# amy-leaf/Recommender-System-using-Apache-Spark-MLlib-

Hardware: AMD Instinct MI355X
Metric: ratings/sec per ALS iteration (rank 64) (higher is better)
Workload: dtype f32-grade (split-f16 x3 MFMA, fp32 accumulate)

## Files before the change

recommender-system-using-apache-spark-mllib-_amd/csrc/gram_solve.hip:

```cpp
#include "als_common.h"
#include "task_order.h"

#include <algorithm>
#include <utility>

namespace als {

typedef float floatx4 __attribute__((ext_vector_type(4)));

constexpr int kYtyTasks = 512;
__host__ __device__ inline int64_t yty_chunk(int64_t n) {
  const int64_t c = (n + kYtyTasks - 1) / kYtyTasks;
  return c < 32 ? 32 : (c + 31) / 32 * 32;
}
constexpr int kRescueGrid = 64;
constexpr float kCondMax = 32.f;
constexpr float kCondMaxImplicit = 8.f;
constexpr int kMaxRank = 128;

template <int CN>
struct Cfg {
  static constexpr int KP = 16 * CN;
  static constexpr int NT = CN * (CN + 1) / 2;
  static constexpr int NP = KP * (KP + 1) / 2;
// ... 302 lines not shown
    const float c1 = alpha * fabsf(rv);
    w = v ? sc * __builtin_sqrtf(c1) : 0.f;
    b = (v && rv > 0.f) ? 1.f + c1 : 0.f;
  } else {
    w = v ? sc : 0.f;
    b = v ? rv : 0.f;
  }
  st_c[lane] = ci;
  st_w[lane] = w;
  st_b[lane] = b;
}

template <int CN, class TS>
__device__ __forceinline__ void split_issue(SplitStep<TS::NC>& s, const int* __restrict__ st_c,
                                            int h, const float* __restrict__ Y, int ld, int d0,
                                            int k) {
  const int q = (threadIdx.x & 63) >> 4;
  const int o = 32 * h + 8 * q;
  const int4 c0 = *reinterpret_cast<const int4*>(st_c + o);
  const int4 c1 = *reinterpret_cast<const int4*>(st_c + o + 4);
  const int ids[8] = {c0.x, c0.y, c0.z, c0.w, c1.x, c1.y, c1.z, c1.w};
#pragma unroll
  for (int j = 0; j < 8; ++j)
    TS::load_clamped(Y + (int64_t)(ids[j] >= 0 ? ids[j] : 0) * ld, s.y[j], d0, ld);
}

template <class TS, bool IMPLICIT>
__device__ __forceinline__ void split_prepare(const SplitStep<TS::NC>& s,
                                              const float* __restrict__ st_w,
                                              const float* __restrict__ st_b, int h,
                                              uint32_t (&hi)[TS::NC][4], uint32_t (&lo)[TS::NC][4],
                                              float (&bf)[TS::NRA]) {
  const int o = 32 * h + 8 * ((threadIdx.x & 63) >> 4);
  const float4 w0 = *reinterpret_cast<const float4*>(st_w + o);
  const float4 w1 = *reinterpret_cast<const float4*>(st_w + o + 4);
  const float4 b0 = *reinterpret_cast<const float4*>(st_b + o);
  const float4 b1 = *reinterpret_cast<const float4*>(st_b + o + 4);
  const float w[8] = {w0.x, w0.y, w0.z, w0.w, w1.x, w1.y, w1.z, w1.w};
  const float b[8] = {b0.x, b0.y, b0.z, b0.w, b1.x, b1.y, b1.z, b1.w};
#pragma unroll
  for (int c = 0; c < TS::NR; ++c)
#pragma unroll
    for (int j = 0; j < 8; ++j) bf[c] = fmaf(b[j], s.y[j][c], bf[c]);
#pragma unroll
  for (int c = 0; c < TS::NC; ++c)
#pragma unroll
    for (int p = 0; p < 4; ++p)
      split_pair_w(s.y[2 * p][c], w[2 * p], s.y[2 * p + 1][c], w[2 * p + 1], hi[c][p], lo[c][p]);
}

template <class TS>
__device__ __forceinline__ void split_mfma(const uint32_t (&hi)[TS::NC][4],
                                           const uint32_t (&lo)[TS::NC][4],
                                           floatx4 (&acc)[TS::N]) {
  static_for<TS::N>([&](auto ti) {
    constexpr int tt = decltype(ti)::value;
    constexpr int a = TS::l1(tt), b = TS::l2(tt);
    const half8v ha = as_h8(hi[a]), hb = as_h8(hi[b]);
    acc[tt] = __builtin_amdgcn_mfma_f32_16x16x32_f16(ha, hb, acc[tt], 0, 0, 0);
    acc[tt] = __builtin_amdgcn_mfma_f32_16x16x32_f16(ha, as_h8(lo[b]), acc[tt], 0, 0, 0);
    acc[tt] = __builtin_amdgcn_mfma_f32_16x16x32_f16(as_h8(lo[a]), hb, acc[tt], 0, 0, 0);
  });
}

template <int CN, bool IMPLICIT, class TS = FullTiles<CN>>
__device__ __forceinline__ void gram_accumulate_split(
    const int32_t* __restrict__ col, const float* __restrict__ val, int64_t pb, int64_t pe,
    const float* __restrict__ Y, int ld, int k, float alpha, float sc,
    floatx4 (&acc)[TS::N], float (&bf)[TS::NRA], int& npos, int* __restrict__ st) {
  const int lane = threadIdx.x & 63, m = lane & 15;
  const int d0 = m * CN;
  int* st_c = st;
  float* st_w = reinterpret_cast<float*>(st + 64);
  float* st_b = reinterpret_cast<float*>(st + 128);
  if (pe <= pb) return;
  auto load_idx = [&](int64_t base, int& ci, float& rv) {
    ci = -1;
    rv = 0.f;
    if (base + lane < pe) {
      ci = col[base + lane];
      rv = val[base + lane];
    }
  };
  const int64_t n = pe - pb;
  const int nsteps = (int)((n + 31) >> 5);
  int ci_n, ci_c;
  float rv_n, rv_c;
  load_idx(pb, ci_c, rv_c);
  load_idx(pb + 64, ci_n, rv_n);
  stage_weights<IMPLICIT>(st_c, st_w, st_b, ci_c, rv_c, sc, alpha);
  if constexpr (IMPLICIT) npos += __popcll(__ballot(ci_c >= 0 && rv_c > 0.f));
  wave_lds_sync();
  SplitStep<TS::NC> sA;
  split_issue<CN, TS>(sA, st_c, 0, Y, ld, d0, k);
  float bp[TS::NRA];
#pragma unroll
  for (int c = 0; c < TS::NRA; ++c) bp[c] = 0.f;
  for (int s = 0; s < nsteps; ++s) {
    uint32_t hi[TS::NC][4], lo[TS::NC][4];
    split_prepare<TS, IMPLICIT>(sA, st_w, st_b, s & 1, hi, lo, bp);
    const int s1 = s + 1;
    if (s1 < nsteps) {
      if ((s1 & 1) == 0) {
        stage_weights<IMPLICIT>(st_c, st_w, st_b, ci_n, rv_n, sc, alpha);
        if constexpr (IMPLICIT) npos += __popcll(__ballot(ci_n >= 0 && rv_n > 0.f));
        wave_lds_sync();
        load_idx(pb + 64 * (int64_t)((s1 >> 1) + 1), ci_n, rv_n);
      }
      split_issue<CN, TS>(sA, st_c, s1 & 1, Y, ld, d0, k);
    }
    split_mfma<TS>(hi, lo, acc);
    if (s & 1) {
#pragma unroll
      for (int c = 0; c < TS::NRA; ++c) {
        bf[c] += bp[c];
        bp[c] = 0.f;
      }
    }
  }
#pragma unroll
  for (int c = 0; c < TS::NRA; ++c) bf[c] += bp[c];
}

__device__ __forceinline__ uint32_t split_word(float t) {
  const _Float16 h = (_Float16)t;
  const _Float16 l = (_Float16)(t - (float)h);
  return (uint32_t)__builtin_bit_cast(unsigned short, h) |
         ((uint32_t)__builtin_bit_cast(unsigned short, l) << 16);
}

template <int NC>
struct PreStep {
  uint32_t w[8][NC];
  uint32_t r[8];
};

template <class TS>
__device__ __forceinline__ void pre_issue(PreStep<TS::NC>& s, const int* __restrict__ st_c,
                                          const uint32_t* __restrict__ st_r, int h,
                                          const uint32_t* __restrict__ base, uint32_t kp) {
  const int q = (threadIdx.x & 63) >> 4;
  const int o = 32 * h + 8 * q;
  const int4 c0 = *reinterpret_cast<const int4*>(st_c + o);
  const int4 c1 = *reinterpret_cast<const int4*>(st_c + o + 4);
  const uint4 r0 = *reinterpret_cast<const uint4*>(st_r + o);
  const uint4 r1 = *reinterpret_cast<const uint4*>(st_r + o + 4);
  const int ids[8] = {c0.x, c0.y, c0.z, c0.w, c1.x, c1.y, c1.z, c1.w};
  s.r[0] = r0.x; s.r[1] = r0.y; s.r[2] = r0.z; s.r[3] = r0.w;
  s.r[4] = r1.x; s.r[5] = r1.y; s.r[6] = r1.z; s.r[7] = r1.w;
#pragma unroll
  for (int j = 0; j < 8; ++j) TS::load_pre(base + (uint64_t)(uint32_t)ids[j] * kp, s.w[j]);
}

template <class TS>
__device__ __forceinline__ void pre_operands(const PreStep<TS::NC>& s, uint32_t rsel,
                                             uint32_t (&hi)[TS::NC][4], uint32_t (&lo)[TS::NC][4],
                                             uint32_t (&rb)[4]) {
#pragma unroll
  for (int c = 0; c < TS::NC; ++c)
#pragma unroll
    for (int p = 0; p < 4; ++p) {
      hi[c][p] = __builtin_amdgcn_perm(s.w[2 * p + 1][c], s.w[2 * p][c], 0x05040100u);
      lo[c][p] = __builtin_amdgcn_perm(s.w[2 * p + 1][c], s.w[2 * p][c], 0x07060302u);
    }
#pragma unroll
  for (int p = 0; p < 4; ++p) rb[p] = __builtin_amdgcn_perm(s.r[2 * p + 1], s.r[2 * p], rsel);
}

template <class TS>
__device__ __forceinline__ void pin_operands(uint32_t (&hi)[TS::NC][4], uint32_t (&lo)[TS::NC][4],
                                             uint32_t (&rb)[4]) {
#pragma unroll
  for (int c = 0; c < TS::NC; ++c)
#pragma unroll
    for (int p = 0; p < 4; ++p) asm volatile("" : "+v"(hi[c][p]), "+v"(lo[c][p]));
  if constexpr (TS::NR > 0) {
#pragma unroll
    for (int p = 0; p < 4; ++p) asm volatile("" : "+v"(rb[p]));
  }
  asm volatile("" ::: "memory");
}

template <class TS>
__device__ __forceinline__ void pre_mfma(const uint32_t (&hi)[TS::NC][4],
                                         const uint32_t (&lo)[TS::NC][4], const uint32_t (&rb)[4],
                                         floatx4 (&acc)[TS::N], floatx4 (&accb)[TS::NRA]) {
  split_mfma<TS>(hi, lo, acc);
  const half8v b = as_h8(rb);
#pragma unroll
  for (int c = 0; c < TS::NR; ++c) {
    accb[c] = __builtin_amdgcn_mfma_f32_16x16x32_f16(as_h8(hi[c]), b, accb[c], 0, 0, 0);
    accb[c] = __builtin_amdgcn_mfma_f32_16x16x32_f16(as_h8(lo[c]), b, accb[c], 0, 0, 0);
  }
}

template <class TS>
__device__ __forceinline__ void gram_accumulate_pre(
    const int32_t* __restrict__ col, const float* __restrict__ val, int64_t pb, int64_t pe,
    const uint32_t* __restrict__ Ysp, uint32_t kp, int zero_row, float sr, int d0,
    floatx4 (&acc)[TS::N], floatx4 (&accb)[TS::NRA], int* __restrict__ st, float& rmax) {
  const int lane = threadIdx.x & 63, m = lane & 15;
  int* st_c = st;
  uint32_t* st_r = reinterpret_cast<uint32_t*>(st + 64);
  if (pe <= pb) return;
  const uint32_t rsel = m == 0 ? 0x05040100u : (m == 1 ? 0x07060302u : 0x0C0C0C0Cu);
  const uint32_t* base = Ysp + d0;
  auto load_idx = [&](int64_t b, int& ci, float& rv) {
    ci = zero_row;
    rv = 0.f;
    if (b + lane < pe) {
      ci = col[b + lane];
      rv = val[b + lane];
    }
  };
  auto stage = [&](int ci, float rv) {
    st_c[lane] = ci;
    st_r[lane] = split_word(sr * rv);
    rmax = fmaxf(rmax, __builtin_fabsf(rv));
    wave_lds_sync();
  };
  const int nsteps = (int)((pe - pb + 31) >> 5);
  int ci, ci_n;
  float rv, rv_n;
  load_idx(pb, ci, rv);
  load_idx(pb + 64, ci_n, rv_n);
  stage(ci, rv);
  PreStep<TS::NC> s;
  pre_issue<TS>(s, st_c, st_r, 0, base, kp);
  for (int t = 0; t < nsteps; ++t) {
    uint32_t hi[TS::NC][4], lo[TS::NC][4], rb[4];
    pre_operands<TS>(s, rsel, hi, lo, rb);
    pin_operands<TS>(hi, lo, rb);
    if (t & 1) {
      stage(ci_n, rv_n);
      load_idx(pb + 64 * (int64_t)((t >> 1) + 2), ci_n, rv_n);
    }
    pre_issue<TS>(s, st_c, st_r, (t + 1) & 1, base, kp);
    pre_mfma<TS>(hi, lo, rb, acc, accb);
  }
}

template <class TS>
__device__ __forceinline__ void gram_accumulate_pre2(
    const int32_t* __restrict__ col, const float* __restrict__ val, int64_t pb, int64_t pe,
    const uint32_t* __restrict__ Ysp, uint32_t kp, int zero_row, float sr, int d0,
    floatx4 (&acc)[TS::N], floatx4 (&accb)[TS::NRA], int* __restrict__ st, float& rmax) {
  const int lane = threadIdx.x & 63, m = lane & 15;
  if (pe <= pb) return;
  const uint32_t rsel = m == 0 ? 0x05040100u : (m == 1 ? 0x07060302u : 0x0C0C0C0Cu);
  const uint32_t* base = Ysp + d0;
  auto load_idx = [&](int64_t b, int& ci, float& rv) {
    ci = zero_row;
    rv = 0.f;
    if (b + lane < pe) {
      ci = col[b + lane];
      rv = val[b + lane];
    }
  };
  auto stage = [&](int slot, int ci, float rv) {
    st[128 * slot + lane] = ci;
    reinterpret_cast<uint32_t*>(st + 128 * slot + 64)[lane] = split_word(sr * rv);
    rmax = fmaxf(rmax, __builtin_fabsf(rv));
    wave_lds_sync();
  };
  auto issue = [&](PreStep<TS::NC>& s, int step) {
    const int slot = (step >> 1) & 1;
    pre_issue<TS>(s, st + 128 * slot, reinterpret_cast<const uint32_t*>(st + 128 * slot + 64),
                  step & 1, base, kp);
  };
  const int nsteps = (int)((pe - pb + 31) >> 5);
  int ci0, ci1, ci_n;
  float rv0, rv1, rv_n;
  load_idx(pb, ci0, rv0);
  load_idx(pb + 64, ci1, rv1);
  load_idx(pb + 128, ci_n, rv_n);
  stage(0, ci0, rv0);
  stage(1, ci1, rv1);
  PreStep<TS::NC> s0, s1;
  issue(s0, 0);
  issue(s1, 1);
  auto body = [&](PreStep<TS::NC>& s, int t) {
    uint32_t hi[TS::NC][4], lo[TS::NC][4], rb[4];
    pre_operands<TS>(s, rsel, hi, lo, rb);
    pin_operands<TS>(hi, lo, rb);
    if (t & 1) {
      stage((t >> 1) & 1, ci_n, rv_n);
      load_idx(pb + 64 * (int64_t)((t >> 1) + 3), ci_n, rv_n);
    }
    issue(s, t + 2);
    pre_mfma<TS>(hi, lo, rb, acc, accb);
  };
  for (int t = 0; t < nsteps; t += 2) {
    body(s0, t);
    if (t + 1 < nsteps) body(s1, t + 1);
  }
}

template <class TS>
__device__ __forceinline__ void rhs_from_tiles(const floatx4 (&accb)[TS::NRA], float scale,
                                               float (&bt)[TS::NRA]) {
  const int lane = threadIdx.x & 63, q = lane >> 4, m = lane & 15;
  const int src = (m >> 2) << 4;
  const int rr = m & 3;
#pragma unroll
  for (int c = 0; c < TS::NRA; ++c) {
    float v[4];
#pragma unroll
    for (int r = 0; r < 4; ++r) v[r] = __shfl(accb[c][r] + __shfl_xor(accb[c][r], 1), src);
    const float x = rr == 0 ? v[0] : (rr == 1 ? v[1] : (rr == 2 ? v[2] : v[3]));
    bt[c] = (c < TS::NR && q == 0) ? x * scale : 0.f;
  }
}

__global__ __launch_bounds__(256) void split_table_kernel(const float* __restrict__ Y,
                                                          int64_t n_src, int ld, int k,
                                                          int kp4_shift,
                                                          const float* __restrict__ scal,
                                                          uint4* __restrict__ Ysp) {
  const float sy = ldexpf(1.f, split_exponent(scal[0]));
  const int64_t total = (n_src + 1) << kp4_shift;
  for (int64_t i = (int64_t)blockIdx.x * 256 + threadIdx.x; i < total;
       i += (int64_t)gridDim.x * 256) {
    const int64_t row = i >> kp4_shift;
    const int d = 4 * (int)(i & ((1 << kp4_shift) - 1));
    float4 v = make_float4(0.f, 0.f, 0.f, 0.f);
    if (row < n_src && d + 4 <= ld) v = *reinterpret_cast<const float4*>(Y + row * ld + d);
    uint4 w;
    w.x = d + 0 < k ? split_word(sy * v.x) : 0u;
    w.y = d + 1 < k ? split_word(sy * v.y) : 0u;
    w.z = d + 2 < k ? split_word(sy * v.z) : 0u;
    w.w = d + 3 < k ? split_word(sy * v.w) : 0u;
    Ysp[i] = w;
  }
}

__device__ __forceinline__ void decode_task(int t, int n_chunks, int n_light, int& chunk,
                                            int& light) {
  const int P = n_chunks < n_light ? n_chunks : n_light;
  chunk = -1;
  light = -1;
  if (t < 2 * P) {
    if (t & 1) light = t >> 1;
    else chunk = t >> 1;
  } else if (n_chunks > P) {
    chunk = t - P;
  } else {
    light = t - P;
  }
}

template <int CN>
__device__ __forceinline__ void tile_ij(int c1, int c2, int r, int& i, int& j) {
  const int lane = threadIdx.x & 63, q = lane >> 4, m = lane & 15;
  i = (4 * q + r) * CN + c1;
  j = m * CN + c2;
}

template <int CN, class T>
__device__ __forceinline__ void pack_gram(const double (&a64)[Cfg<CN>::NT][4], T* __restrict__ P) {
  int tt = 0;
#pragma unroll
  for (int c1 = 0; c1 < CN; ++c1) {
#pragma unroll
    for (int c2 = c1; c2 < CN; ++c2) {
#pragma unroll
      for (int r = 0; r < 4; ++r) {
        int i, j;
        tile_ij<CN>(c1, c2, r, i, j);
        const int hi = i > j ? i : j, lo = i > j ? j : i;
        P[hi * (hi + 1) / 2 + lo] = (T)a64[tt][r];
      }
      ++tt;
    }
  }
}

__device__ __forceinline__ float rcp_t(float d) { return __builtin_amdgcn_rcpf(d); }
__device__ __forceinline__ double rcp_t(double d) {
  double y = __builtin_amdgcn_rcp(d);
  y = fma(fma(-d, y, 1.0), y, y);
  return fma(fma(-d, y, 1.0), y, y);
}
__device__ __forceinline__ float readlane_t(float v, int l) {
  return __builtin_bit_cast(float, __builtin_amdgcn_readlane(__builtin_bit_cast(int, v), l));
}
__device__ __forceinline__ double readlane_t(double v, int l) { return readlane_f64(v, l); }

template <int CN>
struct PanelLds {
  static constexpr int NB = CN, NT = CN * (CN + 1) / 2, CS = 18;
  static constexpr int T = 0, Z = NT * 16 * CS, D = Z + 16 * NB, X = D + 16 * NB,
                       SIZE = X + 16 * NB;
};

__host__ __device__ constexpr int tile_index(int nb, int i, int j) {
  return i * nb - i * (i - 1) / 2 + (j - i);
}

template <int CN>
__device__ __forceinline__ void regularise_f32(floatx4 (&A)[Cfg<CN>::NT], float lam, int k) {
  int tt = 0;
#pragma unroll
  for (int c1 = 0; c1 < CN; ++c1) {
#pragma unroll
    for (int c2 = c1; c2 < CN; ++c2) {
      if (c1 == c2) {
#pragma unroll
        for (int r = 0; r < 4; ++r) {
          int i, j;
          tile_ij<CN>(c1, c2, r, i, j);
          if (i == j) A[tt][r] = (i < k) ? A[tt][r] + lam : 1.f;
        }
      }
      ++tt;
    }
  }
}

template <int P>
__device__ __forceinline__ float gate_above(float x) {
  float r;
  uint64_t m;
  asm volatile("s_lshl_b64 %1, -1, %2\n\ts_nop 0\n\tv_cndmask_b32_e64 %0, 0, %3, %1"
               : "=v"(r), "=&s"(m)
               : "i"(P + 1), "v"(x));
  return r;
}

template <int P>
__device__ __forceinline__ float put_lane(float v, float s) {
  asm volatile("s_nop 1\n\tv_writelane_b32 %0, %1, %2" : "+v"(v) : "s"(s), "i"(P));
  return v;
}

template <int N>
__device__ __forceinline__ void pivot_broadcast(const float (&R)[N], float rb, int p,
                                                float (&a)[N], float& bp) {
  const int addr = p << 2;
#pragma unroll
  for (int i = p; i < N; ++i)
    a[i] = __builtin_bit_cast(float,
                              __builtin_amdgcn_ds_bpermute(addr, __builtin_bit_cast(int, R[i])));
  bp = __builtin_bit_cast(float, __builtin_amdgcn_ds_bpermute(addr, __builtin_bit_cast(int, rb)));
}

template <int N>
__device__ __forceinline__ void pivot_update(float (&R)[N], const float (&a)[N], int p, float f) {
  const float2v nf = {-f, -f};
#pragma unroll
  for (int i = (p + 1) & ~1; i < N; i += 2) {
    const float2v r = __builtin_elementwise_fma((float2v){a[i], a[i + 1]}, nf,
                                                (float2v){R[i], R[i + 1]});
    R[i] = r[0];
    R[i + 1] = r[1];
// ... 653 lines not shown
  });
  bool fin = true;
#pragma unroll
  for (int c = 0; c < NB; ++c) fin = fin && (xcol[c] - xcol[c] == 0.f);
  rmin = fminf(rmin, dpp_f<0xB1>(rmin));
  rmax = fmaxf(rmax, dpp_f<0xB1>(rmax));
  rmin = fminf(rmin, dpp_f<0x4E>(rmin));
  rmax = fmaxf(rmax, dpp_f<0x4E>(rmax));
  rmin = fminf(rmin, dpp_f<0x141>(rmin));
  rmax = fmaxf(rmax, dpp_f<0x141>(rmax));
  rmin = fminf(rmin, dpp_f<0x140>(rmin));
  rmax = fmaxf(rmax, dpp_f<0x140>(rmax));
  return dmin > 0.f && rmin > 0.f && rmax <= cond_max * rmin && __ballot(!fin) == 0;
}

template <int NB, bool SPLIT = kW1SplitSchur<NB>>
__device__ __forceinline__ bool w1_solve(floatx4 (&A)[NB * (NB + 1) / 2], float (&bcol)[NB],
                                         float* __restrict__ lds, int k,
                                         float* __restrict__ xrow, int ld,
                                         float cond_max = kCondMax) {
  float xcol[NB];
  const bool ok = w1_solve_x<NB, SPLIT>(A, bcol, lds, k, xcol, cond_max);
  const int lane = threadIdx.x & 63, m = lane & 15;
  if (lane < 16) {
#pragma unroll
    for (int c = 0; c < NB; ++c) {
      const int d = m * NB + c;
      if (d < ld) xrow[d] = (d < k && ok) ? xcol[c] : 0.f;
    }
  }
  return ok;
}

constexpr int kIrSteps = 3;
constexpr float kIrConv = 3e-4f;
constexpr float kIrDiverge = 0.1f;

struct IrArgs {
  const int32_t* col;
  const float* val;
  const float* Y;
  int64_t pb, pe;
  float alpha;
};

template <int CN>
struct IrLds {
  static constexpr int XS = PanelLds<CN>::SIZE, GS = XS + 128, CC = GS + 128, RV = CC + 64,
                       DX = RV + 16 * CN, SIZE = DX + 16 * CN;
  static_assert(XS % 4 == 0, "fp64 alignment");
};

__device__ __forceinline__ double implicit_residual(const IrArgs& a, int ld, int k,
                                                    const double* __restrict__ yty, double lam_n,
                                                    const double* __restrict__ xs,
                                                    double* __restrict__ gs, int* __restrict__ cc) {
  const int lane = threadIdx.x & 63;
  double r = 0.0;
  for (int64_t base = a.pb; base < a.pe; base += 64) {
    const int nb = (int)(a.pe - base < 64 ? a.pe - base : 64);
    double g = 0.0;
    int c = 0;
    if (lane < nb) {
      c = a.col[base + lane];
      const double rv = (double)a.val[base + lane];
      const float* y = a.Y + (int64_t)c * ld;
      double s0 = 0.0, s1 = 0.0;
      for (int d = 0; d < k; d += 4) {
        const float4 v = *reinterpret_cast<const float4*>(y + d);
        s0 = fma((double)v.x, xs[d], s0);
        s1 = fma((double)v.y, xs[d + 1], s1);
        s0 = fma((double)v.z, xs[d + 2], s0);
        s1 = fma((double)v.w, xs[d + 3], s1);
      }
      const double c1 = (double)a.alpha * fabs(rv);
      g = (rv > 0.0 ? 1.0 + c1 : 0.0) - c1 * (s0 + s1);
    }
    gs[lane] = g;
    cc[lane] = c;
    wave_lds_sync();
    if (lane < k) {
#pragma unroll 8
      for (int j = 0; j < nb; ++j) r = fma(gs[j], (double)a.Y[(int64_t)cc[j] * ld + lane], r);
    }
    wave_lds_sync();
  }
  if (lane < k) {
    for (int e = 0; e < k; ++e) {
      const int hi = lane > e ? lane : e, lo = lane > e ? e : lane;
      r = fma(-yty[hi * (hi + 1) / 2 + lo], xs[e], r);
    }
    r = fma(-lam_n, xs[lane], r);
  }
  return r;
}

template <int CN>
__device__ __forceinline__ bool panel_refine(float* __restrict__ lds, const IrArgs& a, int ld,
                                             int k, const double* __restrict__ yty,
                                             double lam_n) {
  typedef PanelLds<CN> Lo;
  typedef IrLds<CN> Ir;
  float* Xv = lds + Lo::X;
  float* Zv = lds + Lo::Z;
  const float* Dv = lds + Lo::D;
  double* xs = reinterpret_cast<double*>(lds + Ir::XS);
  double* gs = reinterpret_cast<double*>(lds + Ir::GS);
  int* cc = reinterpret_cast<int*>(lds + Ir::CC);
  float* Rv = lds + Ir::RV;
  float* DX = lds + Ir::DX;
  const int lane = threadIdx.x & 63;
  const int pl = (lane % CN) * 16 + lane / CN;
  bool conv = false;
  for (int it = 0; it < kIrSteps; ++it) {
    xs[lane] = lane < k ? (double)Xv[pl] : 0.0;
    wave_lds_sync();
    const double r = implicit_residual(a, ld, k, yty, lam_n, xs, gs, cc);
    if (lane < 16 * CN) Rv[pl] = lane < k ? (float)r : 0.f;
    wave_lds_sync();
    block_fwd_subst<Lo::CS>(CN, lds + Lo::T, Rv, Zv);
    block_back_subst<Lo::CS>(CN, lds + Lo::T, Zv, Dv, DX);
    float nd = 0.f, nx = 0.f;
    if (lane < 16 * CN) {
      const float dx = DX[lane];
      const float xn = Xv[lane] + dx;
      Xv[lane] = xn;
      nd = dx * dx;
      nx = xn * xn;
    }
    wave_lds_sync();
    for (int o = 32; o > 0; o >>= 1) {
      nd += __shfl_xor(nd, o);
      nx += __shfl_xor(nx, o);
    }
    if (nd <= (kIrConv * kIrConv) * nx) {
      conv = true;
      break;
    }
    if (!(nd <= (kIrDiverge * kIrDiverge) * nx)) break;
  }
  return conv;
}

template <int CN, bool IMPLICIT = false>
struct SmemBytes {
  static constexpr int value =
      (int)sizeof(float) * (IMPLICIT ? IrLds<CN>::SIZE : PanelLds<CN>::SIZE);
};
template <bool IMPLICIT>
struct SmemBytes<8, IMPLICIT> {
  static constexpr int value = (int)sizeof(float) * W1Lds::SIZE;
};

__device__ __forceinline__ float shfl_xor_t(float v, int m) { return __shfl_xor(v, m); }
__device__ __forceinline__ double shfl_xor_t(double v, int m) { return shfl_xor_f64(v, m); }

template <int CN, bool IMPLICIT, class AccT>
__device__ __forceinline__ void finish_and_solve(AccT (&tot)[Cfg<CN>::NT][4], AccT (&bt)[CN],
                                                 int64_t n_reg, unsigned char* smem, int k,
                                                 float reg, const double* __restrict__ yty,
                                                 float* __restrict__ xrow, int ld, int row,
                                                 RescueList rl, const IrArgs& ir) {
  constexpr int NT = Cfg<CN>::NT;
  float bq[CN];
  const int m = threadIdx.x & 15;
#pragma unroll
  for (int c = 0; c < CN; ++c) {
    AccT v = bt[c];
    v += shfl_xor_t(v, 16);
    v += shfl_xor_t(v, 32);
    bq[c] = m * CN + c < k ? (float)v : 0.f;
  }
  floatx4 A[NT];
  int tt = 0;
#pragma unroll
  for (int c1 = 0; c1 < CN; ++c1) {
#pragma unroll
    for (int c2 = c1; c2 < CN; ++c2) {
#pragma unroll
      for (int r = 0; r < 4; ++r) {
        if constexpr (IMPLICIT) {
          int i, j;
          tile_ij<CN>(c1, c2, r, i, j);
          const int hi = i > j ? i : j, lo = i > j ? j : i;
          A[tt][r] = (float)((double)tot[tt][r] + yty[hi * (hi + 1) / 2 + lo]);
        } else {
          A[tt][r] = (float)tot[tt][r];
        }
        int i, j;
        tile_ij<CN>(c1, c2, r, i, j);
        if (i >= k || j >= k) A[tt][r] = 0.f;
      }
      ++tt;
    }
  }
  regularise_f32<CN>(A, (float)((double)reg * (double)n_reg), k);
  float* lds = reinterpret_cast<float*>(smem);
  if constexpr (IMPLICIT) {
    bool ok = panel_ldl_solve<CN, false, false>(A, bq, lds, k, xrow, ld);
    if (ok) ok = panel_refine<CN>(lds, ir, ld, k, yty, (double)reg * (double)n_reg);
    panel_store_x<CN>(lds + PanelLds<CN>::X, k, ok, xrow, ld);
    if (!ok) rescue_append(rl, row);
  } else {
    const bool ok = panel_ldl_solve<CN>(A, bq, lds, k, xrow, ld);
    if (!ok) rescue_append(rl, row);
  }
}

template <int N, int NRA>
struct Slot {
  static constexpr int SIZE = (N * 4 + NRA + 1) * 64;
};

template <int N, int NRA, class AccT>
__device__ __forceinline__ void store_slot(double* __restrict__ slot, const AccT (&tot)[N][4],
                                           const AccT (&bt)[NRA], float npos) {
  const int lane = threadIdx.x & 63;
#pragma unroll
  for (int t = 0; t < N; ++t)
#pragma unroll
    for (int r = 0; r < 4; ++r) slot[(t * 4 + r) * 64 + lane] = (double)tot[t][r];
#pragma unroll
  for (int c = 0; c < NRA; ++c) slot[(N * 4 + c) * 64 + lane] = (double)bt[c];
  slot[(N * 4 + NRA) * 64 + lane] = (double)npos;
}

template <int N, int NRA>
__device__ __forceinline__ void add_slot(const double* __restrict__ slot, double (&a64)[N][4],
                                         double (&b64)[NRA], int& npos) {
  const int lane = threadIdx.x & 63;
#pragma unroll
  for (int t = 0; t < N; ++t)
#pragma unroll
    for (int r = 0; r < 4; ++r) a64[t][r] += slot[(t * 4 + r) * 64 + lane];
#pragma unroll
  for (int c = 0; c < NRA; ++c) b64[c] += slot[(N * 4 + c) * 64 + lane];
  npos += (int)slot[(N * 4 + NRA) * 64 + lane];
}

template <int N, int NRA>
__device__ __forceinline__ void store_slot_f32(float* __restrict__ slot, const float (&tot)[N][4],
                                               const float (&bt)[NRA], float npos) {
  const int lane = threadIdx.x & 63;
#pragma unroll
  for (int t = 0; t < N; ++t)
#pragma unroll
    for (int r = 0; r < 4; ++r) slot[(t * 4 + r) * 64 + lane] = tot[t][r];
#pragma unroll
  for (int c = 0; c < NRA; ++c) slot[(N * 4 + c) * 64 + lane] = bt[c];
  slot[(N * 4 + NRA) * 64 + lane] = npos;
}

template <int N, int NRA>
__device__ __forceinline__ void add_slot_f32(const float* __restrict__ slot, double (&a64)[N][4],
                                             double (&b64)[NRA], int& npos) {
  const int lane = threadIdx.x & 63;
#pragma unroll
  for (int t = 0; t < N; ++t)
#pragma unroll
    for (int r = 0; r < 4; ++r) a64[t][r] += (double)slot[(t * 4 + r) * 64 + lane];
#pragma unroll
  for (int c = 0; c < NRA; ++c) b64[c] += (double)slot[(N * 4 + c) * 64 + lane];
  npos += (int)slot[(N * 4 + NRA) * 64 + lane];
}

template <int N, int NRA, class AccT>
__device__ __forceinline__ void zero_acc(AccT (&tot)[N][4], AccT (&bt)[NRA]) {
#pragma unroll
  for (int t = 0; t < N; ++t)
#pragma unroll
    for (int r = 0; r < 4; ++r) tot[t][r] = AccT(0);
#pragma unroll
  for (int c = 0; c < NRA; ++c) bt[c] = AccT(0);
}

template <bool ADD_YTY, int NB = kW1NB, bool SPLIT = kW1SplitSchur<NB>>
__device__ __forceinline__ void w1_finish_and_solve(floatx4 (&A)[NB * (NB + 1) / 2],
                                                    float scale, float (&bt)[NB], int64_t n_reg,
                                                    const float* __restrict__ ytyC,
                                                    unsigned char* smem, int k, float reg,
                                                    float* __restrict__ xrow, int ld, int row,
                                                    RescueList rl, float cond_max = kCondMax);

template <int CN, bool IMPLICIT>
__global__ __launch_bounds__(64, IMPLICIT ? 2 : 3) void gram_solve_kernel(
    const int64_t* __restrict__ row_ptr, const int32_t* __restrict__ col,
    const float* __restrict__ val, const int32_t* __restrict__ light_rows,
    const int32_t* __restrict__ chunk_row, const int64_t* __restrict__ chunk_begin,
    const int64_t* __restrict__ chunk_end, int32_t n_chunks, int32_t n_light,
    const float* __restrict__ Y, float* __restrict__ X, int ld, int k, float reg, float alpha,
    const double* __restrict__ yty, float* __restrict__ slots, int32_t* __restrict__ status,
    const float* __restrict__ scal, const uint32_t* __restrict__ Ysp, int32_t kp,
    int32_t zero_row, RescueList rl) {
  constexpr int NT = Cfg<CN>::NT;
  __shared__ __attribute__((aligned(16))) unsigned char smem[SmemBytes<CN, IMPLICIT>::value];
  floatx4 acc[NT];
#pragma unroll
  for (int t = 0; t < NT; ++t) acc[t] = floatx4{0.f, 0.f, 0.f, 0.f};
  float tot[NT][4], bt[CN];
#pragma unroll
  for (int c = 0; c < CN; ++c) bt[c] = 0.f;
  int npos = 0;
  int chunk, light;
  if constexpr (!IMPLICIT && CN == 4) decode_task_merged(blockIdx.x, n_chunks, n_light, chunk, light);
  else decode_task(blockIdx.x, n_chunks, n_light, chunk, light);
  int64_t pb, pe;
  int row = -1;
  if (chunk >= 0) {
    pb = chunk_begin[chunk];
    pe = chunk_end[chunk];
  } else {
    row = light_rows[light];
    pb = row_ptr[row];
    pe = row_ptr[row + 1];
  }
  float inv2;
  float rmax = 0.f;
  if constexpr (IMPLICIT) {
    const int e = split_exponent(scal[0] * __builtin_sqrtf(alpha * scal[1]));
    inv2 = ldexpf(1.f, -2 * e);
    gram_accumulate_split<CN, true>(col, val, pb, pe, Y, ld, k, alpha, ldexpf(1.f, e), acc, bt,
                                    npos, reinterpret_cast<int*>(smem));
  } else {
    const int ey = split_exponent(scal[0]), er = split_exponent(scal[1]);
    inv2 = ldexpf(1.f, -2 * ey);
    floatx4 accb[CN];
#pragma unroll
    for (int c = 0; c < CN; ++c) accb[c] = floatx4{0.f, 0.f, 0.f, 0.f};
    gram_accumulate_pre<FullTiles<CN>>(col, val, pb, pe, Ysp, (uint32_t)kp, zero_row,
                                       ldexpf(1.f, er), (threadIdx.x & 15) * CN, acc, accb,
                                       reinterpret_cast<int*>(smem), rmax);
    rhs_from_tiles<FullTiles<CN>>(accb, ldexpf(1.f, -ey - er), bt);
    rmax *= ldexpf(1.f, er);
    if (chunk < 0 && (window_miss(diag_max_lane<CN>(acc), (float)(pe - pb), rmax) ||
                      rank_deficient_illcond<CN>(acc, inv2, pe - pb, k, reg))) {
      rescue_append(rl, row);
      return;
    }
  }
#pragma unroll
  for (int t = 0; t < NT; ++t)
#pragma unroll
    for (int r = 0; r < 4; ++r) tot[t][r] = acc[t][r] * inv2;
  if (chunk >= 0) {
    store_slot_f32<NT, CN>(slots + (int64_t)chunk * Cfg<CN>::SLOT, tot, bt,
                           IMPLICIT ? (float)npos : rmax);
    return;
  }
  __syncthreads();
  const int64_t n_reg = IMPLICIT ? (int64_t)npos : (pe - pb);
  if constexpr (!IMPLICIT && CN == 4) {
    static_assert(W1LdsT<4>::SIZE <= PanelLds<4>::SIZE, "W1<4> LDS");
    w1_finish_and_solve<false, 4, false>(acc, inv2, bt, n_reg, nullptr, smem, k, reg,
                                  X + (int64_t)row * ld, ld, row, rl);
  } else {
    finish_and_solve<CN, IMPLICIT, float>(tot, bt, n_reg, smem, k, reg, yty,
                                          X + (int64_t)row * ld, ld, row, rl,
                                          IrArgs{col, val, Y, pb, pe, alpha});
  }
}

__device__ __forceinline__ void block_absmax_publish(float m, unsigned* __restrict__ out) {
  for (int o = 32; o > 0; o >>= 1) m = fmaxf(m, __shfl_xor(m, o));
  __shared__ float red[4];
  if ((threadIdx.x & 63) == 0) red[threadIdx.x >> 6] = m;
  __syncthreads();
  if (threadIdx.x == 0) {
    m = fmaxf(fmaxf(red[0], red[1]), fmaxf(red[2], red[3]));
    atomicMax(out, __float_as_uint(m));
  }
}

__global__ __launch_bounds__(256) void absmax_csr_kernel(const int64_t* __restrict__ row_ptr,
                                                         int32_t n_rows,
                                                         const float* __restrict__ val,
                                                         unsigned* __restrict__ out) {
  const int64_t n = row_ptr[n_rows];
  float m = 0.f;
  const int64_t n4 = n >> 2;
  const float4* v4 = reinterpret_cast<const float4*>(val);
  auto fold = [&](const float4& v) {
    m = fmaxf(m, fmaxf(fmaxf(fabsf(v.x), fabsf(v.y)), fmaxf(fabsf(v.z), fabsf(v.w))));
  };
  const int64_t stride = (int64_t)gridDim.x * 256;
  int64_t i = (int64_t)blockIdx.x * 256 + threadIdx.x;
  for (; i + 3 * stride < n4; i += 4 * stride) {
    const float4 a = v4[i], b = v4[i + stride], c = v4[i + 2 * stride], d = v4[i + 3 * stride];
    fold(a);
    fold(b);
    fold(c);
    fold(d);
  }
  for (; i < n4; i += stride) fold(v4[i]);
  if (blockIdx.x == 0 && threadIdx.x < (n & 3)) m = fmaxf(m, fabsf(val[4 * n4 + threadIdx.x]));
  block_absmax_publish(m, out);
}

__global__ __launch_bounds__(256) void absmax_kernel(const float* __restrict__ x, int64_t n,
                                                     unsigned* __restrict__ out,
                                                     unsigned* __restrict__ zero_word) {
  if (zero_word != nullptr && blockIdx.x == 0 && threadIdx.x < 2) zero_word[threadIdx.x] = 0u;
  float m = 0.f;
  const int64_t n4 = n >> 2;
  const float4* x4 = reinterpret_cast<const float4*>(x);
  auto fold = [&](const float4& v) {
    m = fmaxf(m, fmaxf(fmaxf(fabsf(v.x), fabsf(v.y)), fmaxf(fabsf(v.z), fabsf(v.w))));
  };
  const int64_t stride = (int64_t)gridDim.x * 256;
  int64_t i = blockIdx.x * 256 + threadIdx.x;
  for (; i + 3 * stride < n4; i += 4 * stride) {
    const float4 a = x4[i], b = x4[i + stride], c = x4[i + 2 * stride], d = x4[i + 3 * stride];
    fold(a);
    fold(b);
    fold(c);
    fold(d);
  }
  for (; i < n4; i += stride) fold(x4[i]);
  if (blockIdx.x == 0 && threadIdx.x < (n & 3)) m = fmaxf(m, fabsf(x[4 * n4 + threadIdx.x]));
  block_absmax_publish(m, out);
}

struct SlotRange {
  int s0, n1, t0, n;
  __device__ __forceinline__ int at(int i) const { return i < n1 ? s0 + i : t0 + (i - n1); }
  __device__ __forceinline__ int home() const { return at(0); }
};
__device__ __forceinline__ SlotRange slot_range(const int32_t* __restrict__ sb,
                                                const int32_t* __restrict__ sb2, int h) {
  SlotRange r;
  r.s0 = sb[h];
  r.n1 = sb[h + 1] - r.s0;
  r.t0 = sb2 ? sb2[h] : 0;
  r.n = r.n1 + (sb2 ? sb2[h + 1] - r.t0 : 0);
  return r;
}

template <int SLOT, bool IMPLICIT>
__global__ __launch_bounds__(256) void heavy_sum_f64_kernel(const int32_t* __restrict__ slot_begin,
                                                            const int32_t* __restrict__ slot_begin2,
                                                            float* __restrict__ slots) {
  const int h = blockIdx.y;
  const int e = blockIdx.x * 256 + threadIdx.x;
  if (e >= SLOT) return;
  const SlotRange sr = slot_range(slot_begin, slot_begin2, h);
  if (sr.n <= 1) return;
  const int64_t home = (int64_t)sr.home() * SLOT + e;
  if (!IMPLICIT && e >= SLOT - 64) {
    float mx = 0.f;
    for (int i = 0; i < sr.n; ++i) mx = fmaxf(mx, slots[(int64_t)sr.at(i) * SLOT + e]);
    slots[home] = mx;
    return;
  }
  double a0 = 0.0, a1 = 0.0, a2 = 0.0, a3 = 0.0;
  int i = 0;
  for (; i + 4 <= sr.n; i += 4) {
    a0 += (double)slots[(int64_t)sr.at(i) * SLOT + e];
    a1 += (double)slots[(int64_t)sr.at(i + 1) * SLOT + e];
    a2 += (double)slots[(int64_t)sr.at(i + 2) * SLOT + e];
    a3 += (double)slots[(int64_t)sr.at(i + 3) * SLOT + e];
  }
  for (; i < sr.n; ++i) a0 += (double)slots[(int64_t)sr.at(i) * SLOT + e];
  slots[home] = (float)((a0 + a1) + (a2 + a3));
}

template <int CN, bool IMPLICIT>
__global__ __launch_bounds__(64, 2) void reduce_solve_kernel(
    const int64_t* __restrict__ row_ptr, const int32_t* __restrict__ col,
    const float* __restrict__ val, const float* __restrict__ Y, float alpha,
    const int32_t* __restrict__ heavy_rows, const int32_t* __restrict__ slot_begin,
    const int32_t* __restrict__ slot_begin2, const float* __restrict__ slots,
    float* __restrict__ X, int ld, int k, float reg, const double* __restrict__ yty,
    int32_t* __restrict__ status, const float* __restrict__ scal,
    RescueList rl) {
  constexpr int NT = Cfg<CN>::NT;
  __shared__ __attribute__((aligned(16))) unsigned char smem[SmemBytes<CN, IMPLICIT>::value];
  const int h = blockIdx.x;
  const int row = heavy_rows[h];
  double a64[NT][4], b64[CN];
  zero_acc<NT, CN, double>(a64, b64);
  int npos = 0;
  const float* sl =
      slots + (int64_t)slot_range(slot_begin, slot_begin2, h).home() * Cfg<CN>::SLOT;
  add_slot_f32<NT, CN>(sl, a64, b64, npos);
  const int64_t n_reg = IMPLICIT ? (int64_t)npos : (row_ptr[row + 1] - row_ptr[row]);
  if constexpr (!IMPLICIT) {
    const float s2 = ldexpf(1.f, 2 * split_exponent(scal[0]));
    float d = 0.f;
    const int lane = threadIdx.x & 63, q = lane >> 4, m = lane & 15;
#pragma unroll
    for (int c = 0; c < CN; ++c)
#pragma unroll
      for (int r = 0; r < 4; ++r)
        if (4 * q + r == m) d = fmaxf(d, (float)a64[tile_index(CN, c, c)][r] * s2);
    if (window_miss(d, (float)n_reg, (float)sl[(NT * 4 + CN) * 64 + lane])) {
      rescue_append(rl, row);
      return;
    }
  }
  finish_and_solve<CN, IMPLICIT, double>(a64, b64, n_reg, smem, k, reg, yty,
                                         X + (int64_t)row * ld, ld, row, rl,
                                         IrArgs{col, val, Y, row_ptr[row], row_ptr[row + 1],
                                                alpha});
}

constexpr int kW1NT = 36;
// ... 983 lines not shown
```

Before: 13.68 billion.

## Pack rank-64 RHS into one MFMA tile and raise fused kernel occupancy

For the rank-64 explicit path, the right-hand side accumulation now lands in a single 16x16 MFMA tile instead of four. The rating-weighted operand is masked per column group and used as the A operand, and the reduction step is adjusted to match. This cuts accumulator registers. The LDS allocation is shrunk to the larger of the W1 solve buffer and the staging area, and launch bounds ask for 4 waves. Together these aim for higher occupancy, at the cost of a more intricate lane mapping in the RHS extraction.

```diff
diff --git a/recommender-system-using-apache-spark-mllib-_amd/csrc/gram_solve.hip b/recommender-system-using-apache-spark-mllib-_amd/csrc/gram_solve.hip
--- a/recommender-system-using-apache-spark-mllib-_amd/csrc/gram_solve.hip
+++ b/recommender-system-using-apache-spark-mllib-_amd/csrc/gram_solve.hip
@@ -478,6 +478,12 @@
   for (int j = 0; j < 8; ++j) TS::load_pre(base + (uint64_t)(uint32_t)ids[j] * kp, s.w[j]);
 }
 
+template <class TS, bool ONE>
+struct RhsTiles {
+  static_assert(!ONE || (TS::NR >= 1 && 2 * TS::NR <= 16), "rows 2c, 2c + 1 of one tile");
+  static constexpr int N = ONE ? 1 : TS::NRA;
+};
+
 template <class TS>
 __device__ __forceinline__ void pre_operands(const PreStep<TS::NC>& s, uint32_t rsel,
                                              uint32_t (&hi)[TS::NC][4], uint32_t (&lo)[TS::NC][4],
@@ -507,29 +513,53 @@
   asm volatile("" ::: "memory");
 }
 
-template <class TS>
+template <class TS, bool ONE = false>
 __device__ __forceinline__ void pre_mfma(const uint32_t (&hi)[TS::NC][4],
                                          const uint32_t (&lo)[TS::NC][4], const uint32_t (&rb)[4],
-                                         floatx4 (&acc)[TS::N], floatx4 (&accb)[TS::NRA]) {
+                                         floatx4 (&acc)[TS::N],
+                                         floatx4 (&accb)[RhsTiles<TS, ONE>::N]) {
   split_mfma<TS>(hi, lo, acc);
-  const half8v b = as_h8(rb);
-#pragma unroll
-  for (int c = 0; c < TS::NR; ++c) {
-    accb[c] = __builtin_amdgcn_mfma_f32_16x16x32_f16(as_h8(hi[c]), b, accb[c], 0, 0, 0);
-    accb[c] = __builtin_amdgcn_mfma_f32_16x16x32_f16(as_h8(lo[c]), b, accb[c], 0, 0, 0);
-  }
-}
-
-template <class TS>
+  if constexpr (ONE) {
+    const int m = threadIdx.x & 15;
+#pragma unroll
+    for (int c = 0; c < TS::NR; ++c) {
+      uint32_t rc[4];
+#pragma unroll
+      for (int p = 0; p < 4; ++p) rc[p] = (m >> 1) == c ? rb[p] : 0u;
+      const half8v a = as_h8(rc);
+      accb[0] = __builtin_amdgcn_mfma_f32_16x16x32_f16(a, as_h8(hi[c]), accb[0], 0, 0, 0);
+      accb[0] = __builtin_amdgcn_mfma_f32_16x16x32_f16(a, as_h8(lo[c]), accb[0], 0, 0, 0);
+    }
+  } else {
+    const half8v b = as_h8(rb);
+#pragma unroll
+    for (int c = 0; c < TS::NR; ++c) {
+      accb[c] = __builtin_amdgcn_mfma_f32_16x16x32_f16(as_h8(hi[c]), b, accb[c], 0, 0, 0);
+      accb[c] = __builtin_amdgcn_mfma_f32_16x16x32_f16(as_h8(lo[c]), b, accb[c], 0, 0, 0);
+    }
+  }
+}
+
+template <class TS, bool ONE>
+__device__ __forceinline__ uint32_t pre_rsel() {
+  const int m = threadIdx.x & 15;
+  if constexpr (ONE)
+    return m >= 2 * TS::NR ? 0x0C0C0C0Cu : ((m & 1) ? 0x07060302u : 0x05040100u);
+  else
+    return m == 0 ? 0x05040100u : (m == 1 ? 0x07060302u : 0x0C0C0C0Cu);
+}
+
+template <class TS, bool ONE = false>
 __device__ __forceinline__ void gram_accumulate_pre(
     const int32_t* __restrict__ col, const float* __restrict__ val, int64_t pb, int64_t pe,
     const uint32_t* __restrict__ Ysp, uint32_t kp, int zero_row, float sr, int d0,
-    floatx4 (&acc)[TS::N], floatx4 (&accb)[TS::NRA], int* __restrict__ st, float& rmax) {
-  const int lane = threadIdx.x & 63, m = lane & 15;
+    floatx4 (&acc)[TS::N], floatx4 (&accb)[RhsTiles<TS, ONE>::N], int* __restrict__ st,
+    float& rmax) {
+  const int lane = threadIdx.x & 63;
   int* st_c = st;
   uint32_t* st_r = reinterpret_cast<uint32_t*>(st + 64);
   if (pe <= pb) return;
-  const uint32_t rsel = m == 0 ? 0x05040100u : (m == 1 ? 0x07060302u : 0x0C0C0C0Cu);
+  const uint32_t rsel = pre_rsel<TS, ONE>();
   const uint32_t* base = Ysp + d0;
   auto load_idx = [&](int64_t b, int& ci, float& rv) {
     ci = zero_row;
@@ -562,7 +592,7 @@
       load_idx(pb + 64 * (int64_t)((t >> 1) + 2), ci_n, rv_n);
     }
     pre_issue<TS>(s, st_c, st_r, (t + 1) & 1, base, kp);
-    pre_mfma<TS>(hi, lo, rb, acc, accb);
+    pre_mfma<TS, ONE>(hi, lo, rb, acc, accb);
   }
 }
 
@@ -571,9 +601,9 @@
     const int32_t* __restrict__ col, const float* __restrict__ val, int64_t pb, int64_t pe,
     const uint32_t* __restrict__ Ysp, uint32_t kp, int zero_row, float sr, int d0,
     floatx4 (&acc)[TS::N], floatx4 (&accb)[TS::NRA], int* __restrict__ st, float& rmax) {
-  const int lane = threadIdx.x & 63, m = lane & 15;
+  const int lane = threadIdx.x & 63;
   if (pe <= pb) return;
-  const uint32_t rsel = m == 0 ? 0x05040100u : (m == 1 ? 0x07060302u : 0x0C0C0C0Cu);
+  const uint32_t rsel = pre_rsel<TS, false>();
   const uint32_t* base = Ysp + d0;
   auto load_idx = [&](int64_t b, int& ci, float& rv) {
     ci = zero_row;
@@ -622,10 +652,18 @@
   }
 }
 
-template <class TS>
-__device__ __forceinline__ void rhs_from_tiles(const floatx4 (&accb)[TS::NRA], float scale,
-                                               float (&bt)[TS::NRA]) {
+template <class TS, bool ONE = false>
+__device__ __forceinline__ void rhs_from_tiles(const floatx4 (&accb)[RhsTiles<TS, ONE>::N],
+                                               float scale, float (&bt)[TS::NRA]) {
   const int lane = threadIdx.x & 63, q = lane >> 4, m = lane & 15;
+  if constexpr (ONE) {
+#pragma unroll
+    for (int c = 0; c < TS::NRA; ++c) {
+      const float x = __shfl(accb[0][(2 * c) & 3] + accb[0][((2 * c) & 3) + 1], m + 16 * (c >> 1));
+      bt[c] = (c < TS::NR && q == 0) ? x * scale : 0.f;
+    }
+    return;
+  }
   const int src = (m >> 2) << 4;
   const int rr = m & 3;
 #pragma unroll
@@ -1585,6 +1623,23 @@
   static constexpr int value = (int)sizeof(float) * W1Lds::SIZE;
 };
 
+constexpr int kPreStageWords = 128;
+template <int CN, bool IMPLICIT>
+struct FusedSmemBytes : SmemBytes<CN, IMPLICIT> {};
+template <>
+struct FusedSmemBytes<4, false> {
+  static constexpr int value =
+      (int)sizeof(float) * (W1LdsT<4>::SIZE > kPreStageWords ? W1LdsT<4>::SIZE : kPreStageWords);
+  static_assert(value >= (int)sizeof(float) * W1LdsT<4>::SIZE &&
+                    value >= (int)sizeof(float) * kPreStageWords && value % 16 == 0,
+                "rank 33-64 explicit: Gram staging and W1<4> solve");
+  static_assert(value <= 10240, "rank 33-64 explicit: 16 workgroups per CU");
+};
+template <int CN, bool IMPLICIT>
+constexpr int kFusedWaves = IMPLICIT ? 2 : (CN == 4 ? 4 : 3);
+template <int CN>
+constexpr bool kOneRhsTile = CN == 4;
+
 __device__ __forceinline__ float shfl_xor_t(float v, int m) { return __shfl_xor(v, m); }
 __device__ __forceinline__ double shfl_xor_t(double v, int m) { return shfl_xor_f64(v, m); }
 
@@ -1716,7 +1771,7 @@
                                                     RescueList rl, float cond_max = kCondMax);
 
 template <int CN, bool IMPLICIT>
-__global__ __launch_bounds__(64, IMPLICIT ? 2 : 3) void gram_solve_kernel(
+__global__ __launch_bounds__(64, (kFusedWaves<CN, IMPLICIT>)) void gram_solve_kernel(
     const int64_t* __restrict__ row_ptr, const int32_t* __restrict__ col,
     const float* __restrict__ val, const int32_t* __restrict__ light_rows,
     const int32_t* __restrict__ chunk_row, const int64_t* __restrict__ chunk_begin,
@@ -1726,7 +1781,7 @@
     const float* __restrict__ scal, const uint32_t* __restrict__ Ysp, int32_t kp,
     int32_t zero_row, RescueList rl) {
   constexpr int NT = Cfg<CN>::NT;
-  __shared__ __attribute__((aligned(16))) unsigned char smem[SmemBytes<CN, IMPLICIT>::value];
+  __shared__ __attribute__((aligned(16))) unsigned char smem[FusedSmemBytes<CN, IMPLICIT>::value];
   floatx4 acc[NT];
 #pragma unroll
   for (int t = 0; t < NT; ++t) acc[t] = floatx4{0.f, 0.f, 0.f, 0.f};
@@ -1757,13 +1812,15 @@
   } else {
     const int ey = split_exponent(scal[0]), er = split_exponent(scal[1]);
     inv2 = ldexpf(1.f, -2 * ey);
-    floatx4 accb[CN];
-#pragma unroll
-    for (int c = 0; c < CN; ++c) accb[c] = floatx4{0.f, 0.f, 0.f, 0.f};
-    gram_accumulate_pre<FullTiles<CN>>(col, val, pb, pe, Ysp, (uint32_t)kp, zero_row,
-                                       ldexpf(1.f, er), (threadIdx.x & 15) * CN, acc, accb,
-                                       reinterpret_cast<int*>(smem), rmax);
-    rhs_from_tiles<FullTiles<CN>>(accb, ldexpf(1.f, -ey - er), bt);
+    constexpr bool ONE = kOneRhsTile<CN>;
+    constexpr int NRT = RhsTiles<FullTiles<CN>, ONE>::N;
+    floatx4 accb[NRT];
+#pragma unroll
+    for (int c = 0; c < NRT; ++c) accb[c] = floatx4{0.f, 0.f, 0.f, 0.f};
+    gram_accumulate_pre<FullTiles<CN>, ONE>(col, val, pb, pe, Ysp, (uint32_t)kp, zero_row,
+                                            ldexpf(1.f, er), (threadIdx.x & 15) * CN, acc, accb,
+                                            reinterpret_cast<int*>(smem), rmax);
+    rhs_from_tiles<FullTiles<CN>, ONE>(accb, ldexpf(1.f, -ey - er), bt);
     rmax *= ldexpf(1.f, er);
     if (chunk < 0 && (window_miss(diag_max_lane<CN>(acc), (float)(pe - pb), rmax) ||
                       rank_deficient_illcond<CN>(acc, inv2, pe - pb, k, reg))) {
@@ -1783,7 +1840,8 @@
   __syncthreads();
   const int64_t n_reg = IMPLICIT ? (int64_t)npos : (pe - pb);
   if constexpr (!IMPLICIT && CN == 4) {
-    static_assert(W1LdsT<4>::SIZE <= PanelLds<4>::SIZE, "W1<4> LDS");
+    static_assert((int)sizeof(float) * W1LdsT<4>::SIZE <= FusedSmemBytes<4, false>::value,
+                  "W1<4> LDS");
     w1_finish_and_solve<false, 4, false>(acc, inv2, bt, n_reg, nullptr, smem, k, reg,
                                   X + (int64_t)row * ld, ld, row, rl);
   } else {
```

New measurement: 14.54 billion, median of 6. 1.06x the previous value.
